# NumericalEarth/Breeze.jl

Hardware: AMD Instinct MI355X
Metric: grid-cells advanced/sec (tendency+Poisson step), 512^3 anelastic (higher is better)
Workload: dtype f64

## Files before the change

breeze.jl_amd/csrc/bz_tendency5.hip:

```cpp
#include <cstdlib>

#include "bz_tendency5_kernels.h"

__global__ void k_pi_dry(DevGrid g, double *__restrict__ pi, int n)
{
    const int t = blockIdx.x * blockDim.x + threadIdx.x;
    if (t >= n) return;
    const int k = t - g.Hz;
    const double q = 0.0, qd = 1.0 - q;
    const double Rm = qd * g.Rd + q * g.Rv;
    const double cpm = qd * g.cpd + q * g.cpv;
    pi[t] = pow(g.p_r[k] / g.pst, Rm / cpm);
}

__global__ void k_lev_rows(DevGrid g, const double *__restrict__ pi, LevRow5 *__restrict__ rows, int n)
{
    const int t = blockIdx.x * blockDim.x + threadIdx.x;
    if (t >= n) return;
    const int k = t - g.Hz;
    LevRow5 r;
    r.rho = g.rho[k]; r.rrho = g.rrho[k]; r.rho_f = g.rho_f[k]; r.rrho_f = g.rrho_f[k];
    r.Ax = g.Ax[k]; r.Ay = g.Ay[k]; r.Vinv_c = g.Vinv_c[k]; r.pi = pi[t];
    r.Vinv_f = g.Vinv_f[k]; r.T_r = g.T_r[k];
    for (int q = 0; q < 6; ++q) r.pad[q] = 0.0;
    rows[t] = r;
}

int bzi_lean_setup(bz_ctx *ctx)
{
    const DevGrid &g = ctx->dg;
    const int n = g.Nz + 2 * g.Hz;
    BZ_HIP(hipMalloc(&ctx->d_pi_dry, n * sizeof(double)));
    hipLaunchKernelGGL(k_pi_dry, dim3((n + 63) / 64), dim3(64), 0, 0, g, ctx->d_pi_dry, n);
    ctx->dg.pi_dry = ColPtr(ctx->d_pi_dry + g.Hz);
    BZ_HIP(hipMalloc(&ctx->d_lev_rows, n * sizeof(LevRow5)));
    hipLaunchKernelGGL(k_lev_rows, dim3((n + 63) / 64), dim3(64), 0, 0, g, ctx->d_pi_dry, (LevRow5 *)ctx->d_lev_rows, n);
    BZ_HIP(hipGetLastError());
    BZ_HIP(hipDeviceSynchronize());
    if (ctx->tune.side_cus > 0 && ctx->tune.side_cus < ctx->num_cus) {
        uint32_t mask[32] = {0};
        const int total = ctx->num_cus, want = ctx->tune.side_cus;
        for (int b = 0; b < want; ++b) {
            const int bit = ctx->tune.side_cu_layout == 1 ? (int)((long long)b * total / want) : b;
            mask[bit >> 5] |= 1u << (bit & 31);
        }
        BZ_HIP(hipExtStreamCreateWithCUMask(&ctx->side_stream, (uint32_t)((total + 31) / 32), mask));
    } else
    BZ_HIP(hipStreamCreateWithFlags(&ctx->side_stream, hipStreamNonBlocking));
    BZ_HIP(hipEventCreateWithFlags(&ctx->ev_fork, hipEventDisableTiming));
    BZ_HIP(hipEventCreateWithFlags(&ctx->ev_join, hipEventDisableTiming));
    ctx->side_scalar = ctx->tune.side_scalar;
    ctx->lean = !ctx->tune.no_lean;
    ctx->lean_xcd = !ctx->tune.no_xcd;
    return BZ_OK;
}

void bzi_lean_teardown(bz_ctx *ctx)
{
    if (ctx->d_pi_dry) hipFree(ctx->d_pi_dry);
    ctx->d_pi_dry = nullptr;
    if (ctx->d_lev_rows) hipFree(ctx->d_lev_rows);
    ctx->d_lev_rows = nullptr;
    if (ctx->d_qstate) hipFree(ctx->d_qstate);
    ctx->d_qstate = nullptr;
    if (ctx->h_qstate) hipHostFree(ctx->h_qstate);
    ctx->h_qstate = nullptr;
    if (ctx->ev_q) hipEventDestroy(ctx->ev_q);
    ctx->ev_q = nullptr;
    if (ctx->side_stream) { hipStreamSynchronize(ctx->side_stream); hipStreamDestroy(ctx->side_stream); ctx->side_stream = nullptr; }
    if (ctx->ev_fork) hipEventDestroy(ctx->ev_fork);
    if (ctx->ev_join) hipEventDestroy(ctx->ev_join);
    ctx->ev_fork = ctx->ev_join = nullptr;
}

static int pick_chunk5(const DevGrid &g, int nlev, int rows_per_block, bool fine = false)
{
    long long tiles = (long long)((g.Nx + 63) / 64) * ((g.Ny + rows_per_block - 1) / rows_per_block);
    const int floor_levels = fine ? 64 : 128;
    long long want = ((fine ? 4096 : 1024) + tiles - 1) / tiles;
    long long maxchunks = nlev / floor_levels > 0 ? nlev / floor_levels : 1;
    if (want > maxchunks) want = maxchunks;
    if (want < 1) want = 1;
    if (tiles * want < 512) {
        long long fill = (512 + tiles - 1) / tiles;
        long long cap = nlev / 8 > 0 ? nlev / 8 : 1;
        if (tiles * cap < 256) cap = nlev / 2 > 0 ? nlev / 2 : 1;
        if (fill > cap) fill = cap;
        if (fill > want) want = fill;
    }
    return (int)((nlev + want - 1) / want);
}

template <int TY>
static int lean_launch(bz_ctx *ctx, const bz_state *s, const bz_prognostic *U0, const bz_prognostic *G, const double *pa,
                       const double *pb, double *oa, double *ob, double dt, double alpha, bool first, int rows, int which)
{
    const DevGrid &g = ctx->dg;
    RKEpilogue E;
    E.mode = first ? 3 : 2; E.dt = dt; E.alpha = alpha; E.oma = 1.0 - alpha;
    Lean5 L;
    L.ru = s->rho_u; L.rv = s->rho_v; L.rw = s->rho_w; L.pa = pa; L.pb = pb; L.oa = oa; L.ob = ob; L.out = nullptr;
    L.T = s->T;
    L.pi_dry = ColPtr(ctx->d_pi_dry + g.Hz);
    L.lev = (const LevRow5 *)ctx->d_lev_rows + g.Hz;
    L.qstate = bzi_moisture_state(ctx);
    const int qh = L.qstate ? ctx->q_host : 2;
    L.mforce = 0; L.cor_f = 0.0; L.Fu = ColPtr(nullptr); L.Fv = ColPtr(nullptr); L.Su = ColPtr(nullptr); L.Sv = ColPtr(nullptr);
// ... 144 lines not shown
```

breeze.jl_amd/csrc/bz_tendency5_kernels.h:

```cpp
#pragma once
#include "bz_internal.h"
#include "bz_weno.h"
#include "bz_tendency4_kernels.h"

#ifndef BZ_KO
#define BZ_KO 0
#endif
#ifndef BZ6_ROTATE_DUTY
#define BZ6_ROTATE_DUTY 0
#endif
#ifndef BZ6_UNROLL2
#define BZ6_UNROLL2 0
#endif
#ifndef BZ6_LDS_BARRIER
#define BZ6_LDS_BARRIER 0
#endif
__device__ __forceinline__ void bz6_barrier()
{
#if BZ6_LDS_BARRIER
    __builtin_amdgcn_fence(__ATOMIC_RELEASE, "workgroup", "local");
    __builtin_amdgcn_s_barrier();
    __builtin_amdgcn_fence(__ATOMIC_ACQUIRE, "workgroup", "local");
#else
    __syncthreads();
#endif
}
typedef long long ix_t;
typedef unsigned ix32_t;

struct LevRow5 {
    double rho, rrho;
    double rho_f, rrho_f;
    double Ax, Ay, Vinv_c;
    double pi;
    double Vinv_f, T_r;
    double pad[6];
};
struct Lev5 {
    const LevRow5 *p;
#ifdef __HIPCC__
    __device__ __forceinline__ double at(int k, int f) const { return ((ColPtr::cptr)(const double *)p)[(long long)k * 16 + f]; }
    __device__ __forceinline__ double rho(int k) const { return at(k, 0); }
    __device__ __forceinline__ double rrho(int k) const { return at(k, 1); }
    __device__ __forceinline__ double rho_f(int k) const { return at(k, 2); }
    __device__ __forceinline__ double rrho_f(int k) const { return at(k, 3); }
    __device__ __forceinline__ double Ax(int k) const { return at(k, 4); }
    __device__ __forceinline__ double Ay(int k) const { return at(k, 5); }
    __device__ __forceinline__ double Vinv_c(int k) const { return at(k, 6); }
    __device__ __forceinline__ double pi(int k) const { return at(k, 7); }
    __device__ __forceinline__ double Vinv_f(int k) const { return at(k, 8); }
    __device__ __forceinline__ double T_r(int k) const { return at(k, 9); }
#endif
};
static_assert(sizeof(LevRow5) == 16 * sizeof(double), "LevRow5 is sixteen reals");

#ifndef BZ_LEAN_WAVES
#define BZ_LEAN_WAVES (sizeof(double) == 8 ? 4 : 6)
#endif
#ifndef BZ5_ZERO_SHORTCUT
#define BZ5_ZERO_SHORTCUT 1
#endif
#ifndef BZ5_TOPS_AHEAD
#define BZ5_TOPS_AHEAD 1
#endif
#ifndef BZ6_W_WAVES
#define BZ6_W_WAVES 4
#endif
#ifndef BZ5_EB
#define BZ5_EB 64
#endif
#ifndef BZ5_RAW_LDS
#define BZ5_RAW_LDS 0
#endif
#ifndef BZ5_SCALAR_WAVES
#define BZ5_SCALAR_WAVES (sizeof(double) == 8 ? 4 : 6)
#endif

struct Lean5 {
    const double *ru, *rv, *rw;
    const double *pa, *pb;
    double *out;
    double *oa, *ob;
    double *T;
    ColPtr pi_dry;
    const LevRow5 *lev;
    int mforce;
    double cor_f;
    ColPtr Fu, Fv;
    ColPtr Su, Sv;
    const double *vel, *bT, *bq;
    const int *qstate;
    int xcd;
    int by0, bys;
};

__device__ __forceinline__ void bz_block5(const Lean5 &L, int &bx, int &by, int &bz)
{
    bx = blockIdx.x; by = blockIdx.y; bz = blockIdx.z;
    if (L.xcd) {
        const unsigned gx = gridDim.x, gy = gridDim.y;
        const unsigned W = gx * gy * gridDim.z;
        unsigned w = bx + gx * (by + gy * bz);
        w = (w & 7u) * (W >> 3) + (w >> 3);
        bx = (int)(w % gx);
        by = (int)((w / gx) % gy);
        bz = (int)(w / (gx * gy));
    }
    by = L.by0 + by * L.bys;
    bx = __builtin_amdgcn_readfirstlane(bx);
    by = __builtin_amdgcn_readfirstlane(by);
    bz = __builtin_amdgcn_readfirstlane(bz);
}

__device__ __forceinline__ void st_img5(double *__restrict__ f, long long n, double v, long long ox, long long oy)
{
    f[n] = v;
    if (ox) f[n + ox] = v;
    if (oy) {
        f[n + oy] = v;
        if (ox) f[n + ox + oy] = v;
    }
}


__device__ __forceinline__ double bz_temperature5(const DevGrid &g, double rth, double rq, int k, const ColPtr pi_dry)
{
    const double rho = g.rho[k], rrho = g.rrho[k];
    const double th = bz_cdiv(rth, rho, rrho), q = bz_cdiv(rq, rho, rrho);
    if (pi_dry.p && __all(q == 0.0)) return pi_dry[k] * th;
    const double qd = 1.0 - q;
    const double cpm = qd * g.cpd + q * g.cpv;
    return bz_exner_factor(g, k, q, cpm) * th;
}

// ... 232 lines not shown
        }
        if (zz) fzb_hi = 0.0;
        else fzb_hi = (BZ_KO & 128) ? rf * (cfz * b[3]) : rf * (cfz * bz_upB(b[1], b[2], b[3], b[4], b[5], tb, lz, Bz));
        }
        double pa_n, pb_n;
        if constexpr (DRYQ) { pa_n = araw[0]; pb_n = b[3]; araw[0] = araw[1]; araw[1] = araw[2]; araw[2] = ta_raw; }
        else if (BZ_KO & 4) { pa_n = a[3]; pb_n = b[3]; }
        else if constexpr (BZ5_RAW_LDS) {
            double *ra = RAW + (lv3 * 2 + 0) * NT + t, *rb = ra + NT;
            pa_n = *ra; pb_n = *rb;
            *ra = ta_raw; *rb = tb_raw;
        } else { pa_n = pa[n]; pb_n = pb[n]; }
        T[buf ^ 1][0][ty + 3][tx + 3] = a[4];
        if constexpr (Q) T[buf ^ 1][1][ty + 3][tx + 3] = b[4];
        {
            const double rh = rho1, rr = rrho1;
            bool z1 = (b[4] == 0.0);
#pragma unroll
            for (int q = 0; q < HPT; ++q)
                if (hok[q]) {
                    T[buf ^ 1][0][hr[q]][hc[q]] = bz_cdiv(ha[q], rh, rr);
                    if constexpr (Q) {
                        const double hbv = bz_cdiv(hb[q], rh, rr);
                        T[buf ^ 1][1][hr[q]][hc[q]] = hbv;
                        z1 = z1 && (hbv == 0.0);
                    }
                }
            if (ZS && !__all(z1) && tx == 0) ZF[(lv3 + 1) % 3] = 0;
        }
        if (!(BZ_KO & 64)) __syncthreads();
        {
            double na = __shfl_down(fxa, 1);
            const double xa = __shfl(ea, src);
            if (tx == le) na = xa;
            const double dya = FY[buf][0][ty + 1][tx] - fya;
            const double Vi = Vi_k;
            const double ga = -(Vi * ((na - fxa) + dya + (fza_hi - fza)));
            double gb = 0.0;
            if constexpr (Q) {
                double nb = __shfl_down(fxb, 1);
                const double xb = __shfl(eb, src);
                if (tx == le) nb = xb;
                const double dyb = FY[buf][1][ty + 1][tx] - fyb;
                gb = -(Vi * ((nb - fxb) + dyb + (fzb_hi - fzb)));
            }
            if (store) {
                const double rth = bz_rk_apply_pre(E.mode, E.dt, E.alpha, E.oma, u0a, E.u0_out, ga, pa_n, n);
                F.oa[n] = rth;
                if constexpr (Q) {
                    const double rq = bz_rk_apply_pre(E.mode, E.dt, E.alpha, E.oma, u0b, E.u0b_out, gb, pb_n, n);
                    F.ob[n] = rq;
                }
            }
        }
        fza = fza_hi; fzb = fzb_hi;
#pragma unroll
        for (int s = 0; s < 5; ++s) { a[s] = a[s + 1]; b[s] = b[s + 1]; }
        a[5] = ta; b[5] = tb;
        buf ^= 1;
    }
}


template <bool DRYQ, bool GUARD>
__device__ __forceinline__ bool bz_lean_skip(const Lean5 &F)
{
    if constexpr (!GUARD) return false;
    const bool dry = F.qstate != nullptr && __builtin_amdgcn_readfirstlane(*F.qstate) == 1;
    return dry != DRYQ;
}
template <int TY, bool WY = false, bool DRYQ = false, bool GUARD = true>
__global__ __launch_bounds__(64 * TY) __attribute__((amdgpu_waves_per_eu(BZ5_SCALAR_WAVES, BZ5_SCALAR_WAVES))) void k5_scalar_pair(DevGrid g, Lean5 F, int kchunk, RKEpilogue E)
{
    constexpr int TR = TY + 6, TC = 72;
    __shared__ double T[2 * 2 * TR * TC];
    __shared__ double FY[2 * 2 * (TY + 1) * 64];
    __shared__ int ZF[3];
    __shared__ double RAW[(!DRYQ && BZ5_RAW_LDS) ? 3 * 2 * 64 * TY : 1];
    if (bz_lean_skip<DRYQ, GUARD>(F)) return;
    k5_scalar_pair_body<TY, WY, DRYQ>(g, F, kchunk, E, T, FY, ZF, RAW);
}

template <int KIND>
__device__ __forceinline__ double flux_x_lean(const DevGrid &g, const Tend3Fields &F, const double *__restrict__ m, int i, int j, int k, int By = 3)
{
    const long long n = g.idx(i, j, k);
    const double a = (KIND == T3_V && By != 3) ? bz_symm2(g.Ax[k] * F.ru[n - g.Sx], g.Ax[k] * F.ru[n]) : adv_x<KIND>(g, F, n, k);
    const double rh = (KIND == T3_W) ? g.rho_f[k] : g.rho[k], rr = (KIND == T3_W) ? g.rrho_f[k] : g.rrho[k];
    if constexpr (KIND == T3_U)
        return a * bz_up5(bz_cdiv(m[n - 2], rh, rr), bz_cdiv(m[n - 1], rh, rr), bz_cdiv(m[n], rh, rr), bz_cdiv(m[n + 1], rh, rr),
                          bz_cdiv(m[n + 2], rh, rr), bz_cdiv(m[n + 3], rh, rr), a > 0.0);
    else
        return a * bz_up5(bz_cdiv(m[n - 3], rh, rr), bz_cdiv(m[n - 2], rh, rr), bz_cdiv(m[n - 1], rh, rr), bz_cdiv(m[n], rh, rr),
                          bz_cdiv(m[n + 1], rh, rr), bz_cdiv(m[n + 2], rh, rr), a > 0.0);
}


template <int TY, bool MF = false, bool WY = false, bool ST = false>
__global__ __launch_bounds__(64 * TY, BZ_LEAN_WAVES) void k6_u(DevGrid g, Lean5 L, int kchunk, RKEpilogue E)
{
    static_assert(!(ST && WY), "stored-velocity instantiations: periodic / slab rows");
    constexpr int TR = TY + 6, TC = 72, NT = 64 * TY;
    constexpr int NH1 = TR * 70 - TY * 64;
    constexpr int NH2 = 3 * (TY + 1) + 64 + 3 * TY;
    static_assert(NH1 <= NT && NH2 <= NT, "one frame cell of each kind per thread");
    __shared__ double U[2][TR][TC];
    __shared__ double RU[2][TY][TC];
    __shared__ double RV[2][TY + 1][TC];
    __shared__ double RW[2][TY][TC];
    __shared__ double FY[2][TY + 1][64];
    int bx, by, bz;
    bz_block5(L, bx, by, bz);
    const int tx = threadIdx.x, ty = threadIdx.y, t = ty * 64 + tx, tc = tx + 3;
    const int i0 = bx * 64, j0 = by * TY;
    const int i = i0 + tx, j = j0 + ty;
    const int ic = min(i, g.Nx + 2), jc = min(j, g.Ny + 2);
    const int ie = i0 - 1, le = 0;
    const int kbeg = bz * kchunk, kend = min(kbeg + kchunk, g.Nz);
    if (kbeg >= kend) return;
    const ix_t sz = (ix_t)g.Sxy;
    const bool store = (i < g.Nx) && (j < g.Ny);
    const double *__restrict__ ru = L.ru, *__restrict__ rv = L.rv, *__restrict__ rw = L.rw;
    const double *__restrict__ vel = ST ? L.vel : L.ru;
    Tend3Fields F;
    F.ru = L.ru; F.rv = L.rv; F.rw = L.rw; F.u = F.v = F.w = F.T = F.q = nullptr; F.c = ST ? L.vel : nullptr; F.G = L.out;
    ix_t n = (ix_t)g.idx(ic, jc, kbeg);
    const bool h1ok = !(BZ_KO & 32768) && t < NH1;
    int h1r = 0, h1c = 0;
    {
        const int h = h1ok ? t : 0;
        if (h < 6 * 70) { const int rr = h / 70; h1c = h - rr * 70; h1r = (rr < 3) ? rr : TY + rr; }
        else { const int hh = h - 6 * 70, rr = hh / 6, cc = hh - rr * 6; h1r = 3 + rr; h1c = (cc < 3) ? cc : 64 + cc; }
    }
    const ix_t h1n = (ix_t)g.idx(min(i0 - 3 + h1c, g.Nx + 2), min(j0 - 3 + h1r, g.Ny + 2), kbeg);
    const bool h1raw = h1ok && h1r >= 3 && h1r < TY + 3 && (h1c == 2 || h1c == 67 || h1c == 68);
    const bool h2ok = !(BZ_KO & 32768) && t < NH2;
    int h2sel = 0, h2r = 0, h2c = 0;
    {
        const int id = h2ok ? t : 0;
        if (id < 3 * (TY + 1)) { h2r = id / 3; const int cc = id - 3 * h2r; h2c = (cc < 2) ? 1 + cc : 67; }
        else if (id < 3 * (TY + 1) + 64) { h2r = TY; h2c = 3 + (id - 3 * (TY + 1)); }
        else { h2sel = 1; const int m = id - 3 * (TY + 1) - 64; h2r = m / 3; const int cc = m - 3 * h2r; h2c = (cc < 2) ? 1 + cc : 67; }
    }
    const double *__restrict__ h2src = h2sel ? rw : rv;
    const ix_t h2n = (ix_t)g.idx(min(i0 - 3 + h2c, g.Nx + 2), min(j0 + h2r, g.Ny + 2), kbeg) + (h2sel ? sz : (ix_t)0);

    double r[6];
#pragma unroll
    for (int s = 0; s < 6; ++s) r[s] = ST ? vel[n + s * sz - 3 * sz] : bz_cdiv(ru[n + s * sz - 3 * sz], g.rho[kbeg + s - 3], g.rrho[kbeg + s - 3]);
    double fz_lo = vflux<T3_U>(g, F, n, kbeg, r[0], r[1], r[2], r[3], r[4], r[5]);
    double q0 = ru[n], q1 = ru[n + sz], q2 = ru[n + 2 * sz];
    U[0][ty + 3][tc] = r[3];
    RU[0][ty][tc] = q0;
    RV[0][ty][tc] = rv[n];
    RW[0][ty][tc] = rw[n + sz];
    if (h1ok) {
        const double raw = (ST && !h1raw) ? 0.0 : ru[h1n];
        U[0][h1r][h1c] = ST ? vel[h1n] : bz_cdiv(raw, g.rho[kbeg], g.rrho[kbeg]);
        if (h1raw) RU[0][h1r - 3][h1c] = raw;
    }
    if (h2ok) { if (h2sel) RW[0][h2r][h2c] = h2src[h2n]; else RV[0][h2r][h2c] = h2src[h2n]; }
    double tcur_raw = ru[n + 3 * sz];
    double tcur_v = ST ? vel[n + 3 * sz] : 0.0;
    double u0cur = (E.mode == 2) ? E.u0[n] : 0.0;
    __syncthreads();

    double edge = 0.0;
    int buf = 0;
#if BZ6_UNROLL2
#pragma unroll 2
#endif
    for (int k = kbeg; k < kend; ++k, n += sz) {
        const ix_t lev1 = (ix_t)(k + 1 - kbeg) * sz;
        const double p_top = ST ? ru[n + sz] : ru[n + ((k + 4 <= g.Nz + g.Hz - 1) ? 4 * sz : 3 * sz)];
        const double p_topv = ST ? vel[n + ((k + 4 <= g.Nz + g.Hz - 1) ? 4 * sz : 3 * sz)] : 0.0;
        const double p_h1 = (BZ_KO & 256) ? p_top : h1ok ? (ST ? vel : ru)[h1n + lev1] : 0.0;
        const double p_h1raw = (ST && h1raw) ? ru[h1n + lev1] : 0.0;
        const double p_h2 = (BZ_KO & 512) ? p_top : h2ok ? h2src[h2n + lev1] : 0.0;
        const double p_rv = (BZ_KO & 1024) ? p_top * 0.5 : rv[n + sz], p_rw = (BZ_KO & 1024) ? p_top * 0.25 : rw[n + 2 * sz];
        const double p_u0 = (BZ_KO & 2048) ? p_top : (E.mode == 2) ? E.u0[n + sz] : 0.0;
        if (((k - kbeg) & (BZ5_EB - 1)) == 0) {
            const int kk = min(k + (tx & (BZ5_EB - 1)), kend - 1);
            edge = ST ? flux_x_at<T3_U>(g, F, ie, jc, kk) : flux_x_lean<T3_U>(g, F, ru, ie, jc, kk);
        }
        const int src = (k - kbeg) & (BZ5_EB - 1);
        const double Ax = g.Ax[k], Ay = g.Ay[k], Az = g.Az;
        const double c0 = r[3];
        const double(*Uk)[TC] = U[buf];
        const double *rur = RU[buf][ty] + tc, *ur = Uk[ty + 3] + tc;
        const double ax = bz_symm4(Ax * rur[-1], Ax * q0, Ax * rur[1], Ax * rur[2]);
        const double fx = ax * bz_up5(ur[-2], ur[-1], c0, ur[1], ur[2], ur[3], ax > 0.0);
        const double *rvr = RV[buf][ty] + tc;
        const double ay = bz_symm4(Ay * rvr[-2], Ay * rvr[-1], Ay * rvr[0], Ay * rvr[1]);
        const double fy = ay * bz_up5y<WY>(Uk[ty][tc], Uk[ty + 1][tc], Uk[ty + 2][tc], c0, Uk[ty + 4][tc], Uk[ty + 5][tc], ay > 0.0, by5_face<WY>(g, __builtin_amdgcn_readfirstlane(j)));
        FY[buf][ty][tx] = fy;
        if (ty == (BZ6_ROTATE_DUTY ? ((k - kbeg) & (TY - 1)) : 0) && !(BZ_KO & 4096)) {
            const double *rvt = RV[buf][TY] + tc;
            const double at = bz_symm4(Ay * rvt[-2], Ay * rvt[-1], Ay * rvt[0], Ay * rvt[1]);
            FY[buf][TY][tx] = at * bz_up5y<WY>(Uk[TY][tc], Uk[TY + 1][tc], Uk[TY + 2][tc], Uk[TY + 3][tc], Uk[TY + 4][tc], Uk[TY + 5][tc], at > 0.0,
                                               by5_face<WY>(g, j0 + TY));
        }
        const double tnew = ST ? tcur_v : bz_cdiv(tcur_raw, g.rho[k + 3], g.rrho[k + 3]);
        const double *rwr = RW[buf][ty] + tc;
        const double wt = bz_symm4(Az * rwr[-2], Az * rwr[-1], Az * rwr[0], Az * rwr[1]);
        const double fz_hi = wt * bz_upB(r[1], r[2], r[3], r[4], r[5], tnew, wt > 0.0, bz_buffer_face(k + 1, g.Nz));
        U[buf ^ 1][ty + 3][tc] = r[4];
        RU[buf ^ 1][ty][tc] = ST ? p_top : q1;
        RV[buf ^ 1][ty][tc] = p_rv;
        RW[buf ^ 1][ty][tc] = p_rw;
        if (h1ok) {
            U[buf ^ 1][h1r][h1c] = ST ? p_h1 : bz_cdiv(p_h1, g.rho[k + 1], g.rrho[k + 1]);
            if (h1raw) RU[buf ^ 1][h1r - 3][h1c] = ST ? p_h1raw : p_h1;
        }
        if (h2ok) { if (h2sel) RW[buf ^ 1][h2r][h2c] = p_h2; else RV[buf ^ 1][h2r][h2c] = p_h2; }
        if (!(BZ_KO & 16384) && (!(BZ_KO & 8192) || ((k - kbeg) & 1))) bz6_barrier();
        {
            double nb = __shfl_up(fx, 1);
            const double e = __shfl(edge, src);
            if (tx == le) nb = e;
            const double dx = fx - nb;
            const double dy = (BZ_KO & 16384) ? 0.5 * fy : FY[buf][ty + 1][tx] - fy;
            double Gu = -(g.Vinv_c[k] * (dx + dy + (fz_hi - fz_lo)));
            if constexpr (MF) {
                if (L.mforce & 1) {
                    const double *rv0 = RV[buf][ty] + tc, *rv1 = RV[buf][ty + 1] + tc;
                    const double a = (rv0[-1] + rv1[-1]) / 2, b = (rv0[0] + rv1[0]) / 2;
                    Gu -= -L.cor_f * ((a + b) / 2);
                }
                if (L.mforce & (2 | 8)) {
                    const double rho = g.rho[k];
                    double tot = (L.mforce & 8) ? rho * L.Su[k] : 0.0;
                    if (L.mforce & 2) tot = (L.mforce & 8) ? tot + rho * L.Fu[k] : rho * L.Fu[k];
                    Gu += tot;
                }
            }
            if (store) L.out[n] = (ST && E.mode == 0) ? Gu : bz_rk_apply_pre(E.mode, E.dt, E.alpha, E.oma, u0cur, E.u0_out, Gu, q0, n);
        }
        fz_lo = fz_hi;
#pragma unroll
        for (int s = 0; s < 5; ++s) r[s] = r[s + 1];
        r[5] = tnew;
        if (ST) q0 = p_top;
        else { q0 = q1; q1 = q2; q2 = tcur_raw; tcur_raw = p_top; }
        u0cur = p_u0;
        if (ST) tcur_v = p_topv;
        buf ^= 1;
    }
}


template <int TY, bool MF = false, bool WY = false, bool ST = false>
__global__ __launch_bounds__(64 * TY, ((MF && WY) ? 4 : BZ_LEAN_WAVES)) void k6_v(DevGrid g, Lean5 L, int kchunk, RKEpilogue E)
{
    static_assert(!(ST && WY), "stored-velocity instantiations: periodic / slab rows");
    constexpr int RV = TY + 6, RM = TY + 4;
    constexpr int TC = 72;
    __shared__ double Tv[2][RV][TC];
    __shared__ double Tm[2][3][RM][64];
    __shared__ double FY[2][TY + 1][64];
    constexpr int NT = 64 * TY, NFR = 16 * 64, HPT = (NFR + NT - 1) / NT;
    int bx, by, bz;
    bz_block5(L, bx, by, bz);
    const int tx = threadIdx.x, ty = threadIdx.y, t = ty * 64 + tx, tc = tx + 3;
    const int i0 = bx * 64, j0 = by * TY;
    const int i = i0 + tx, j = j0 + ty;
    const int ic = min(i, g.Nx + 2), jc = min(j, g.Ny + 2);
    const int nact = min(64, g.Nx - i0);
    const int ie = i0 + nact, le = nact - 1;
    const int kbeg = bz * kchunk, kend = min(kbeg + kchunk, g.Nz);
    if (kbeg >= kend) return;
    const ix_t sz = (ix_t)g.Sxy;
    const bool store = (i < g.Nx) && (j < g.Ny) && !(WY && j == 0);
    const int ju = __builtin_amdgcn_readfirstlane(j);
    const int Bf = by5_face<WY>(g, ju), Bc = by5_center<WY>(g, ju), Bc0 = by5_center<WY>(g, j0 - 1);
    const double *__restrict__ ru = L.ru, *__restrict__ rv = L.rv, *__restrict__ rw = L.rw;
    const double *__restrict__ vel = ST ? L.vel : L.rv;
    Tend3Fields F;
    F.ru = L.ru; F.rv = L.rv; F.rw = L.rw; F.u = F.v = F.w = F.T = F.q = nullptr; F.c = ST ? L.vel : nullptr; F.G = L.out;
    const double Az = g.Az;
    ix_t n = (ix_t)g.idx(ic, jc, kbeg);

    bool hok[HPT];
    int hsel[HPT], hrow[HPT];
    ix_t hn[HPT];
    const double *hsrc[HPT];
#pragma unroll
    for (int q = 0; q < HPT; ++q) {
        const int h = t + q * NT;
        hok[q] = h < NFR;
        const int id = __builtin_amdgcn_readfirstlane(hok[q] ? (h >> 6) : 0);
        int sel, row, grow;
        if (id < 6) { sel = 0; row = (id < 3) ? id : TY + id; grow = j0 - 3 + row; }
        else if (id < 9) { sel = 1; const int m = id - 6; row = (m < 2) ? m : TY + 2; grow = j0 - 2 + row; }
        else if (id < 13) { sel = 2; const int m = id - 9; row = (m < 2) ? m : TY + m; grow = j0 - 2 + row; }
        else { sel = 3; const int m = id - 13; row = (m < 2) ? m : TY + 2; grow = j0 - 2 + row; }
        hsel[q] = sel; hrow[q] = row;
        hsrc[q] = (sel == 1) ? ru : (sel == 3) ? rw : (ST && sel == 0) ? vel : rv;
        hn[q] = (ix_t)g.idx(min(i0 + tx, g.Nx + 2), min(grow, g.Ny + 2), kbeg) + (sel == 3 ? sz : (ix_t)0);
    }
    auto frame_load = [&](int q, ix_t lev) -> double { return hsrc[q][hn[q] + lev]; };
    auto frame_store = [&](int b, int q, double raw, int klev) {
        if (hsel[q] == 0) Tv[b][hrow[q]][tc] = ST ? raw : bz_cdiv(raw, g.rho[klev], g.rrho[klev]);
        else Tm[b][hsel[q] - 1][hrow[q]][tx] = ((hsel[q] == 1) ? g.Ax[klev] : (hsel[q] == 2) ? g.Ay[klev] : Az) * raw;
    };

    const bool sok = t < 5 * TY;
    const int srow = sok ? t / 5 : 0, scc = sok ? t % 5 : 0, scol = (scc < 3) ? scc : 64 + scc;
    const ix_t sn = (ix_t)g.idx(min(i0 - 3 + scol, g.Nx + 2), min(j0 + srow, g.Ny + 2), kbeg);

    double r[6];
#pragma unroll
    for (int s = 0; s < 6; ++s) r[s] = ST ? vel[n + s * sz - 3 * sz] : bz_cdiv(rv[n + s * sz - 3 * sz], g.rho[kbeg + s - 3], g.rrho[kbeg + s - 3]);
    double fz_lo;
    if (WY && Bf != 3) {
        const double wt0 = bz_symm2(Az * rw[n - (ix_t)g.Sx], Az * rw[n]);
        fz_lo = wt0 * bz_upB(r[0], r[1], r[2], r[3], r[4], r[5], wt0 > 0.0, bz_buffer_face(kbeg, g.Nz));
    } else fz_lo = vflux<T3_V>(g, F, n, kbeg, r[0], r[1], r[2], r[3], r[4], r[5]);
    double q0 = rv[n], q1 = rv[n + sz], q2 = rv[n + 2 * sz];
    Tv[0][ty + 3][tc] = r[3];
    if (sok) Tv[0][srow + 3][scol] = ST ? vel[sn] : bz_cdiv(rv[sn], g.rho[kbeg], g.rrho[kbeg]);
    Tm[0][0][ty + 2][tx] = g.Ax[kbeg] * ru[n];
    Tm[0][1][ty + 2][tx] = g.Ay[kbeg] * q0;
    Tm[0][2][ty + 2][tx] = Az * rw[n + sz];
#pragma unroll
    for (int q = 0; q < HPT; ++q)
        if (hok[q]) frame_store(0, q, frame_load(q, 0), kbeg);
    __syncthreads();

    double tcur_raw = rv[n + 3 * sz];
// ... 8 lines not shown
        for (int q = 0; q < HPT; ++q) hnext[q] = hok[q] ? frame_load(q, lev) : 0.0;
        const double p_side = sok ? (ST ? vel : rv)[sn + lev] : 0.0;
        const double p_top = ST ? rv[n + sz] : rv[n + ((k + 4 <= g.Nz + g.Hz - 1) ? 4 * sz : 3 * sz)];
        const double p_topv = ST ? vel[n + ((k + 4 <= g.Nz + g.Hz - 1) ? 4 * sz : 3 * sz)] : 0.0;
        const double p_u0 = (E.mode == 2) ? E.u0[n + sz] : 0.0;
        const double tnew_raw = tcur_raw, u0v = u0cur;
        const double ru_n = g.Ax[k + 1] * ru[n + sz], rw_n = Az * rw[n + 2 * sz];
        double cor_u = 0.0, cg1 = 0.0, cg3 = 0.0;
        if constexpr (MF) { if ((L.mforce & 1) && tx == 63) { const ix_t sy = (ix_t)g.Sx; cg1 = ru[n - sy + 1]; cg3 = ru[n + 1]; } }
        if (((k - kbeg) & (BZ5_EB - 1)) == 0) {
            const int kk = min(k + (tx & (BZ5_EB - 1)), kend - 1);
            edge = ST ? flux_x_at<T3_V>(g, F, ie, jc, kk) : flux_x_lean<T3_V>(g, F, rv, ie, jc, kk, Bf);
        }
        const int src = (k - kbeg) & (BZ5_EB - 1);
        const double rho = g.rho[k];
        const double c0 = r[3];
        const double(*V)[TC] = Tv[buf];
        const double *vrow = V[ty + 3] + tc;
        const double(*MU)[64] = Tm[buf][0];
        const double(*MV)[64] = Tm[buf][1];
        const double(*MW)[64] = Tm[buf][2];
        const double ut = bz_symm4y<WY>(MU[ty][tx], MU[ty + 1][tx], MU[ty + 2][tx], MU[ty + 3][tx], Bf);
        const double fx = ut * bz_up5(vrow[-3], vrow[-2], vrow[-1], c0, vrow[1], vrow[2], ut > 0.0);
        const double vt = (!WY || Bc == 3) ? bz_symm4(MV[ty + 1][tx], MV[ty + 2][tx], MV[ty + 3][tx], MV[ty + 4][tx]) : bz_symm2(MV[ty + 2][tx], MV[ty + 3][tx]);
        const double fy = vt * bz_up5y<WY>(V[ty + 1][tc], V[ty + 2][tc], c0, V[ty + 4][tc], V[ty + 5][tc], V[ty + 6][tc], vt > 0.0, Bc);
        FY[buf][ty + 1][tx] = fy;
        if (ty == 0 && !(BZ_KO & 4096)) {
            const double vb = (!WY || Bc0 == 3) ? bz_symm4(MV[0][tx], MV[1][tx], MV[2][tx], MV[3][tx]) : bz_symm2(MV[1][tx], MV[2][tx]);
            FY[buf][0][tx] = vb * bz_up5y<WY>(V[0][tc], V[1][tc], V[2][tc], V[3][tc], V[4][tc], V[5][tc], vb > 0.0, Bc0);
        }
        const double tnew = ST ? tcur_v : bz_cdiv(tnew_raw, g.rho[k + 3], g.rrho[k + 3]);
        const double wt = bz_symm4y<WY>(MW[ty][tx], MW[ty + 1][tx], MW[ty + 2][tx], MW[ty + 3][tx], Bf);
        const double fz_hi = wt * bz_upB(r[1], r[2], r[3], r[4], r[5], tnew, wt > 0.0, bz_buffer_face(k + 1, g.Nz));
        if constexpr (MF) {
            if (L.mforce & 1) {
                const double Axk = g.Ax[k];
                const double l1 = MU[ty + 1][tx + 1], l3 = MU[ty + 2][tx + 1];
                const double c1 = (tx == 63) ? Axk * cg1 : l1, c3 = (tx == 63) ? Axk * cg3 : l3;
                cor_u = (((MU[ty + 1][tx] + c1) / 2 + (MU[ty + 2][tx] + c3) / 2) / 2) / Axk;
            }
        }
        Tv[buf ^ 1][ty + 3][tc] = r[4];
        if (sok) Tv[buf ^ 1][srow + 3][scol] = ST ? p_side : bz_cdiv(p_side, g.rho[k + 1], g.rrho[k + 1]);
        Tm[buf ^ 1][0][ty + 2][tx] = ru_n;
        Tm[buf ^ 1][1][ty + 2][tx] = g.Ay[k + 1] * (ST ? p_top : q1);
        Tm[buf ^ 1][2][ty + 2][tx] = rw_n;
#pragma unroll
        for (int q = 0; q < HPT; ++q)
            if (hok[q]) frame_store(buf ^ 1, q, hnext[q], k + 1);
        bz6_barrier();
        {
            double nb = __shfl_down(fx, 1);
            const double e = __shfl(edge, src);
            if (tx == le) nb = e;
            const double dx = nb - fx;
            const double dy = fy - FY[buf][ty][tx];
            double Gv = -(g.Vinv_c[k] * (dx + dy + (fz_hi - fz_lo)));
            if constexpr (MF) {
                if (L.mforce & 1) Gv -= L.cor_f * cor_u;
                if (L.mforce & (4 | 16)) {
                    double tot = (L.mforce & 16) ? rho * L.Sv[k] : 0.0;
                    if (L.mforce & 4) tot = (L.mforce & 16) ? tot + rho * L.Fv[k] : rho * L.Fv[k];
                    Gv += tot;
                }
            }
            if (store) L.out[n] = (ST && E.mode == 0) ? Gv : bz_rk_apply_pre(E.mode, E.dt, E.alpha, E.oma, u0v, E.u0_out, Gv, q0, n);
            if constexpr (WY) {
                if (i < g.Nx && j == 0) L.out[n] = 0.0;
                if (i < g.Nx && j == g.Ny - 1) L.out[n + (ix_t)g.Sx] = 0.0;
            }
        }
        fz_lo = fz_hi;
        if (ST) q0 = p_top;
        else { q0 = q1; q1 = q2; q2 = tnew_raw; tcur_raw = p_top; }
        u0cur = p_u0;
        if (ST) tcur_v = p_topv;
#pragma unroll
        for (int s = 0; s < 5; ++s) r[s] = r[s + 1];
        r[5] = tnew;
        buf ^= 1;
    }
}

__device__ __forceinline__ double buoyancy5(const DevGrid &g, double rth, double rq, int k, double rho, double rrho, double pi, double T_ref)
{
    const double th = bz_cdiv(rth, rho, rrho), q = bz_cdiv(rq, rho, rrho);
    double T;
    if (__all(q == 0.0)) T = pi * th;
    else {
        const double qd = 1.0 - q;
        const double cpm = qd * g.cpd + q * g.cpv;
        T = bz_exner_factor(g, k, q, cpm) * th;
    }
    const double Rm = (1.0 - q) * g.Rd + q * g.Rv;
    const double rhop = rho * (g.Rd * T_ref / (Rm * T) - 1.0);
    return -g.g * rhop;
}


template <int TY, bool WY = false, bool DRYQ = false, bool GUARD = true, int BM = 4>
__global__ __launch_bounds__(64 * TY, BZ6_W_WAVES) void k6_w(DevGrid g, Lean5 L, int kchunk, RKEpilogue E)
{
    constexpr bool ST = BM != 4;
    static_assert(!(ST && (WY || DRYQ || GUARD)), "stored-velocity instantiations: periodic / slab rows, no moisture-scan dispatch");
    if (bz_lean_skip<DRYQ, GUARD>(L)) return;
    constexpr int TR = TY + 6, TC = 72, NT = 64 * TY, NH = TR * 70 - TY * 64;
    static_assert(NH <= NT, "one frame cell per thread");
    __shared__ double T[2][TR][TC];
    __shared__ double FY[2][TY + 1][64];
    int bx, by, bz;
    bz_block5(L, bx, by, bz);
    const int tx = threadIdx.x, ty = threadIdx.y, t = ty * 64 + tx, tc = tx + 3;
    const int i0 = bx * 64, j0 = by * TY;
    const int i = i0 + tx, j = j0 + ty;
    const int ic = min(i, g.Nx + 2), jc = min(j, g.Ny + 2);
    const int nact = min(64, g.Nx - i0);
    const int ie = i0 + nact, le = nact - 1;
    const int kbeg = 1 + bz * kchunk, kend = min(kbeg + kchunk, g.Nz);
    if (kbeg >= kend) return;
    const ix32_t sz = (ix32_t)g.Sxy;
    const bool store = (i < g.Nx) && (j < g.Ny);
    const double *__restrict__ ru = L.ru, *__restrict__ rv = L.rv, *__restrict__ rw = L.rw;
    const double *__restrict__ pa = L.pa, *__restrict__ pb = L.pb;
    const double *__restrict__ vel = ST ? L.vel : L.rw;
    const double *__restrict__ bT = L.bT, *__restrict__ bq = L.bq;
    const Lev5 LV{L.lev};
    constexpr bool dryq = DRYQ;
    Tend3Fields F;
    F.ru = L.ru; F.rv = L.rv; F.rw = L.rw; F.u = F.v = F.w = F.T = F.q = nullptr; F.c = ST ? L.vel : nullptr; F.G = L.out;
    const double Az = g.Az;
    ix32_t n = (ix32_t)g.idx(ic, jc, kbeg);
    const bool hok = t < NH;
    int hr = 0, hc = 0;
    {
        const int h = hok ? t : 0;
        if (h < 6 * 70) { const int rr = h / 70; hc = h - rr * 70; hr = (rr < 3) ? rr : TY + rr; }
        else { const int hh = h - 6 * 70, rr = hh / 6, cc = hh - rr * 6; hr = 3 + rr; hc = (cc < 3) ? cc : 64 + cc; }
    }
    const ix32_t hn = (ix32_t)g.idx(min(i0 - 3 + hc, g.Nx + 2), min(j0 - 3 + hr, g.Ny + 2), kbeg);
    const ix32_t ntop0 = (ix32_t)g.idx(ic, min(j0 + TY, g.Ny), kbeg);
    const bool top = (ty == 0);

    double wr[6], qu[4], qv[4], qt[4], qw[4];
    double raw0 = 0.0, raw1 = 0.0, raw2 = 0.0;
#pragma unroll
    for (int s = 0; s < 6; ++s) {
        const double x = rw[n + s * sz - 3 * sz];
        wr[s] = ST ? vel[n + s * sz - 3 * sz] : bz_cdiv(x, LV.rho_f(kbeg + s - 3), LV.rrho_f(kbeg + s - 3));
        if (s >= 1 && s <= 4) qw[s - 1] = Az * x;
        if (s == 3) raw0 = x;
        if (s == 4) raw1 = x;
        if (s == 5) raw2 = x;
    }
#pragma unroll
    for (int s = 0; s < 4; ++s) {
        const int kk = kbeg - 2 + s;
        const double Axk = ST ? g.Ax[kk] : LV.Ax(kk), Ayk = ST ? g.Ay[kk] : LV.Ay(kk);
        qu[s] = Axk * ru[n + s * sz - 2 * sz];
        qv[s] = Ayk * rv[n + s * sz - 2 * sz];
        qt[s] = top ? Ayk * rv[ntop0 + s * sz - 2 * sz] : 0.0;
    }
    double fz_lo, b_lo, r_lo = 0.0;
    {
        const int B = bz_buffer_center(kbeg - 1, g.Nz);
        const double wt = (B == 3) ? bz_symm4(qw[0], qw[1], qw[2], qw[3]) : bz_symm2(qw[1], qw[2]);
        fz_lo = wt * bz_upB(wr[0], wr[1], wr[2], wr[3], wr[4], wr[5], wt > 0.0, B);
        if constexpr (BM == 4) b_lo = buoyancy5(g, pa[n - sz], dryq ? 0.0 : pb[n - sz], kbeg - 1, LV.rho(kbeg - 1), LV.rrho(kbeg - 1), LV.pi(kbeg - 1), LV.T_r(kbeg - 1));
        else if constexpr (BM == 0) b_lo = buoyancy3(g, bT[n - sz], bq[n - sz], kbeg - 1);
        else if constexpr (BM == 3) b_lo = bz_buoyancy(g, bT, bq, (long long)(n - sz), kbeg - 1);
        else if constexpr (BM == 2) { b_lo = bT[n - sz] - g.p_r[kbeg - 1]; r_lo = bq[n - sz] - g.rho[kbeg - 1]; }
        else b_lo = 0.0;
    }
    T[0][ty + 3][tc] = wr[3];
    if (hok) T[0][hr][hc] = ST ? vel[hn] : bz_cdiv(rw[hn], LV.rho_f(kbeg), LV.rrho_f(kbeg));
    double tcur_raw = rw[n + 3 * sz];
    double tcur_v = ST ? vel[n + 3 * sz] : 0.0;
    double u0cur = (E.mode == 2) ? E.u0[n] : 0.0;
    __syncthreads();

    double edge = 0.0;
    int buf = 0;
    for (int k = kbeg; k < kend; ++k, n += sz) {
        const ix32_t lev = (ix32_t)(k - kbeg) * sz;
        const double p_h = hok ? (ST ? vel : rw)[hn + lev + sz] : 0.0;
        const double p_top = rw[n + ((k + 4 <= g.Nz + g.Hz) ? 4 * sz : 3 * sz)];
        const double p_topv = ST ? vel[n + ((k + 4 <= g.Nz + g.Hz) ? 4 * sz : 3 * sz)] : 0.0;
        const double Tcur = (BM == 1) ? 0.0 : (ST ? bT : pa)[n], rqcur = (BM == 1) ? 0.0 : ST ? bq[n] : dryq ? 0.0 : pb[n];
        const double p_u0 = (E.mode == 2) ? E.u0[n + sz] : 0.0;
        const double Axn = ST ? g.Ax[k + 2] : LV.Ax(k + 2), Ayn = ST ? g.Ay[k + 2] : LV.Ay(k + 2);
        const double qun = Axn * ru[n + 2 * sz], qvn = Ayn * rv[n + 2 * sz];
        const double qtn = top ? Ayn * rv[ntop0 + lev + 2 * sz] : 0.0;
        if (((k - kbeg) & (BZ5_EB - 1)) == 0) {
            const int kk = min(k + (tx & (BZ5_EB - 1)), kend - 1);
            edge = ST ? flux_x_at<T3_W>(g, F, ie, jc, kk) : flux_x_lean<T3_W>(g, F, rw, ie, jc, kk);
        }
        const int src = (k - kbeg) & (BZ5_EB - 1);
        const int Bf = bz_buffer_face(k, g.Nz);
        const double w0 = wr[3];
        const double qwnew = Az * (ST ? rw[n + 2 * sz] : raw2);
        const double uold = ST ? rw[n] : raw0;
        const double(*Tk)[TC] = T[buf];
        const double *wrow = Tk[ty + 3] + tc;
        const double ut = (Bf == 3) ? bz_symm4(qu[0], qu[1], qu[2], qu[3]) : bz_symm2(qu[1], qu[2]);
        const double fx = ut * bz_up5(wrow[-3], wrow[-2], wrow[-1], w0, wrow[1], wrow[2], ut > 0.0);
        const double vt = (Bf == 3) ? bz_symm4(qv[0], qv[1], qv[2], qv[3]) : bz_symm2(qv[1], qv[2]);
        const double fy = vt * bz_up5y<WY>(Tk[ty][tc], Tk[ty + 1][tc], Tk[ty + 2][tc], w0, Tk[ty + 4][tc], Tk[ty + 5][tc], vt > 0.0, by5_face<WY>(g, __builtin_amdgcn_readfirstlane(j)));
        FY[buf][ty][tx] = fy;
        if (top && !(BZ_KO & 4096)) {
            const double v2 = (Bf == 3) ? bz_symm4(qt[0], qt[1], qt[2], qt[3]) : bz_symm2(qt[1], qt[2]);
            FY[buf][TY][tx] = v2 * bz_up5y<WY>(Tk[TY][tc], Tk[TY + 1][tc], Tk[TY + 2][tc], Tk[TY + 3][tc], Tk[TY + 4][tc], Tk[TY + 5][tc], v2 > 0.0,
                                               by5_face<WY>(g, j0 + TY));
        }
        const double wnew = ST ? tcur_v : bz_cdiv(tcur_raw, LV.rho_f(k + 3), LV.rrho_f(k + 3));
        double fz_hi;
        {
            const int B = bz_buffer_center(k, g.Nz);
            const double wt = (B == 3) ? bz_symm4(qw[1], qw[2], qw[3], qwnew) : bz_symm2(qw[2], qw[3]);
            fz_hi = wt * bz_upB(wr[1], wr[2], wr[3], wr[4], wr[5], wnew, wt > 0.0, B);
        }
        double b_hi = 0.0, r_hi = 0.0;
        if constexpr (BM == 4) b_hi = buoyancy5(g, Tcur, rqcur, k, LV.rho(k), LV.rrho(k), LV.pi(k), LV.T_r(k));
        else if constexpr (BM == 0) b_hi = buoyancy3(g, Tcur, rqcur, k);
        else if constexpr (BM == 3) b_hi = bz_buoyancy(g, bT, bq, (long long)n, k);
        else if constexpr (BM == 2) { b_hi = Tcur - g.p_r[k]; r_hi = rqcur - g.rho[k]; }
        T[buf ^ 1][ty + 3][tc] = wr[4];
        if (hok) T[buf ^ 1][hr][hc] = ST ? p_h : bz_cdiv(p_h, LV.rho_f(k + 1), LV.rrho_f(k + 1));
        bz6_barrier();
        {
            double nb = __shfl_down(fx, 1);
            const double e = __shfl(edge, src);
            if (tx == le) nb = e;
            const double dx = nb - fx;
            const double dy = FY[buf][ty + 1][tx] - fy;
            const double adv = -((ST ? g.Vinv_f[k] : LV.Vinv_f(k)) * (dx + dy + (fz_hi - fz_lo)));
            double Gval;
            if constexpr (BM == 2) Gval = adv - (b_hi - b_lo) * g.rdzf[k] - g.g * ((r_hi + r_lo) / 2.0);
            else if constexpr (BM == 1) Gval = adv;
            else Gval = adv + 0.5 * (b_lo + b_hi);
            if (store)
                L.out[n] = (ST && E.mode == 0) ? Gval : bz_rk_apply_pre(E.mode, E.dt, E.alpha, E.oma, u0cur, E.u0_out, Gval, uold, n);
        }
        fz_lo = fz_hi;
        b_lo = b_hi;
        r_lo = r_hi;
#pragma unroll
        for (int s = 0; s < 3; ++s) { qu[s] = qu[s + 1]; qv[s] = qv[s + 1]; qt[s] = qt[s + 1]; qw[s] = qw[s + 1]; }
        qu[3] = qun; qv[3] = qvn; qt[3] = qtn; qw[3] = qwnew;
        raw0 = raw1; raw1 = raw2; raw2 = tcur_raw;
        tcur_raw = p_top; u0cur = p_u0;
        if (ST) tcur_v = p_topv;
#pragma unroll
        for (int s = 0; s < 5; ++s) wr[s] = wr[s + 1];
        wr[5] = wnew;
        buf ^= 1;
    }
}
```

Before: 4.191 billion.

## Unroll u-kernel vertical loop by two and specialize dry buoyancy with cached ln(pi)

The u-momentum kernel's vertical sweep is manually unrolled by two for the plain periodic variant. Stencil registers are indexed by phase modulo six and three, so the per-level shift of the r and q windows becomes a rotation once per pair of levels. The buoyancy routine gets a compile-time dry specialization that skips moisture work. The moist path now uses a precomputed ln(pi) column, stored in the padded level row, in place of the Exner factor call, and the edge flux index is derived from the current linear index rather than recomputed. These changes aim to cut register moves and arithmetic, but the unroll may raise register pressure and the mod-indexed arrays rely on full unrolling to stay in registers.

```diff
diff --git a/breeze.jl_amd/csrc/bz_tendency5.hip b/breeze.jl_amd/csrc/bz_tendency5.hip
--- a/breeze.jl_amd/csrc/bz_tendency5.hip
+++ b/breeze.jl_amd/csrc/bz_tendency5.hip
@@ -21,8 +21,8 @@
     LevRow5 r;
     r.rho = g.rho[k]; r.rrho = g.rrho[k]; r.rho_f = g.rho_f[k]; r.rrho_f = g.rrho_f[k];
     r.Ax = g.Ax[k]; r.Ay = g.Ay[k]; r.Vinv_c = g.Vinv_c[k]; r.pi = pi[t];
-    r.Vinv_f = g.Vinv_f[k]; r.T_r = g.T_r[k];
-    for (int q = 0; q < 6; ++q) r.pad[q] = 0.0;
+    r.Vinv_f = g.Vinv_f[k]; r.T_r = g.T_r[k]; r.lnpi = g.lnpi[k];
+    for (int q = 0; q < 5; ++q) r.pad[q] = 0.0;
     rows[t] = r;
 }
 
diff --git a/breeze.jl_amd/csrc/bz_tendency5_kernels.h b/breeze.jl_amd/csrc/bz_tendency5_kernels.h
--- a/breeze.jl_amd/csrc/bz_tendency5_kernels.h
+++ b/breeze.jl_amd/csrc/bz_tendency5_kernels.h
@@ -8,9 +8,6 @@
 #endif
 #ifndef BZ6_ROTATE_DUTY
 #define BZ6_ROTATE_DUTY 0
-#endif
-#ifndef BZ6_UNROLL2
-#define BZ6_UNROLL2 0
 #endif
 #ifndef BZ6_LDS_BARRIER
 #define BZ6_LDS_BARRIER 0
@@ -34,7 +31,8 @@
     double Ax, Ay, Vinv_c;
     double pi;
     double Vinv_f, T_r;
-    double pad[6];
+    double lnpi;
+    double pad[5];
 };
 struct Lev5 {
     const LevRow5 *p;
@@ -50,6 +48,7 @@
     __device__ __forceinline__ double pi(int k) const { return at(k, 7); }
     __device__ __forceinline__ double Vinv_f(int k) const { return at(k, 8); }
     __device__ __forceinline__ double T_r(int k) const { return at(k, 9); }
+    __device__ __forceinline__ double lnpi(int k) const { return at(k, 10); }
 #endif
 };
 static_assert(sizeof(LevRow5) == 16 * sizeof(double), "LevRow5 is sixteen reals");
@@ -448,9 +447,15 @@
 }
 
 template <int KIND>
+__device__ __forceinline__ double flux_x_lean_at(const DevGrid &g, const Tend3Fields &F, const double *__restrict__ m, long long n, int k, int By = 3);
+template <int KIND>
 __device__ __forceinline__ double flux_x_lean(const DevGrid &g, const Tend3Fields &F, const double *__restrict__ m, int i, int j, int k, int By = 3)
 {
-    const long long n = g.idx(i, j, k);
+    return flux_x_lean_at<KIND>(g, F, m, g.idx(i, j, k), k, By);
+}
+template <int KIND>
+__device__ __forceinline__ double flux_x_lean_at(const DevGrid &g, const Tend3Fields &F, const double *__restrict__ m, long long n, int k, int By)
+{
     const double a = (KIND == T3_V && By != 3) ? bz_symm2(g.Ax[k] * F.ru[n - g.Sx], g.Ax[k] * F.ru[n]) : adv_x<KIND>(g, F, n, k);
     const double rh = (KIND == T3_W) ? g.rho_f[k] : g.rho[k], rr = (KIND == T3_W) ? g.rrho_f[k] : g.rrho[k];
     if constexpr (KIND == T3_U)
@@ -515,9 +520,9 @@
 #pragma unroll
     for (int s = 0; s < 6; ++s) r[s] = ST ? vel[n + s * sz - 3 * sz] : bz_cdiv(ru[n + s * sz - 3 * sz], g.rho[kbeg + s - 3], g.rrho[kbeg + s - 3]);
     double fz_lo = vflux<T3_U>(g, F, n, kbeg, r[0], r[1], r[2], r[3], r[4], r[5]);
-    double q0 = ru[n], q1 = ru[n + sz], q2 = ru[n + 2 * sz];
+    double q[3] = {ru[n], ru[n + sz], ru[n + 2 * sz]};
     U[0][ty + 3][tc] = r[3];
-    RU[0][ty][tc] = q0;
+    RU[0][ty][tc] = q[0];
     RV[0][ty][tc] = rv[n];
     RW[0][ty][tc] = rw[n + sz];
     if (h1ok) {
@@ -533,10 +538,12 @@
 
     double edge = 0.0;
     int buf = 0;
-#if BZ6_UNROLL2
-#pragma unroll 2
-#endif
-    for (int k = kbeg; k < kend; ++k, n += sz) {
+    constexpr int GL = (!MF && !WY && !ST) ? 2 : 1;
+    for (int k0 = kbeg; k0 < kend; k0 += GL) {
+#pragma unroll
+    for (int ph = 0; ph < GL; ++ph) {
+        const int k = k0 + ph;
+        if (k >= kend) break;
         const ix_t lev1 = (ix_t)(k + 1 - kbeg) * sz;
         const double p_top = ST ? ru[n + sz] : ru[n + ((k + 4 <= g.Nz + g.Hz - 1) ? 4 * sz : 3 * sz)];
         const double p_topv = ST ? vel[n + ((k + 4 <= g.Nz + g.Hz - 1) ? 4 * sz : 3 * sz)] : 0.0;
@@ -551,10 +558,10 @@
         }
         const int src = (k - kbeg) & (BZ5_EB - 1);
         const double Ax = g.Ax[k], Ay = g.Ay[k], Az = g.Az;
-        const double c0 = r[3];
+        const double c0 = r[(3 + ph) % 6];
         const double(*Uk)[TC] = U[buf];
         const double *rur = RU[buf][ty] + tc, *ur = Uk[ty + 3] + tc;
-        const double ax = bz_symm4(Ax * rur[-1], Ax * q0, Ax * rur[1], Ax * rur[2]);
+        const double ax = bz_symm4(Ax * rur[-1], Ax * q[ph % 3], Ax * rur[1], Ax * rur[2]);
         const double fx = ax * bz_up5(ur[-2], ur[-1], c0, ur[1], ur[2], ur[3], ax > 0.0);
         const double *rvr = RV[buf][ty] + tc;
         const double ay = bz_symm4(Ay * rvr[-2], Ay * rvr[-1], Ay * rvr[0], Ay * rvr[1]);
@@ -569,9 +576,9 @@
         const double tnew = ST ? tcur_v : bz_cdiv(tcur_raw, g.rho[k + 3], g.rrho[k + 3]);
         const double *rwr = RW[buf][ty] + tc;
         const double wt = bz_symm4(Az * rwr[-2], Az * rwr[-1], Az * rwr[0], Az * rwr[1]);
-        const double fz_hi = wt * bz_upB(r[1], r[2], r[3], r[4], r[5], tnew, wt > 0.0, bz_buffer_face(k + 1, g.Nz));
-        U[buf ^ 1][ty + 3][tc] = r[4];
-        RU[buf ^ 1][ty][tc] = ST ? p_top : q1;
+        const double fz_hi = wt * bz_upB(r[(1 + ph) % 6], r[(2 + ph) % 6], r[(3 + ph) % 6], r[(4 + ph) % 6], r[(5 + ph) % 6], tnew, wt > 0.0, bz_buffer_face(k + 1, g.Nz));
+        U[buf ^ 1][ty + 3][tc] = r[(4 + ph) % 6];
+        RU[buf ^ 1][ty][tc] = ST ? p_top : q[(1 + ph) % 3];
         RV[buf ^ 1][ty][tc] = p_rv;
         RW[buf ^ 1][ty][tc] = p_rw;
         if (h1ok) {
@@ -600,17 +607,28 @@
                     Gu += tot;
                 }
             }
-            if (store) L.out[n] = (ST && E.mode == 0) ? Gu : bz_rk_apply_pre(E.mode, E.dt, E.alpha, E.oma, u0cur, E.u0_out, Gu, q0, n);
+            if (store) L.out[n] = (ST && E.mode == 0) ? Gu : bz_rk_apply_pre(E.mode, E.dt, E.alpha, E.oma, u0cur, E.u0_out, Gu, q[ph % 3], n);
         }
         fz_lo = fz_hi;
-#pragma unroll
-        for (int s = 0; s < 5; ++s) r[s] = r[s + 1];
-        r[5] = tnew;
-        if (ST) q0 = p_top;
-        else { q0 = q1; q1 = q2; q2 = tcur_raw; tcur_raw = p_top; }
+        r[ph % 6] = tnew;
+        if (ST) q[(1 + ph) % 3] = p_top;
+        else { q[ph % 3] = tcur_raw; tcur_raw = p_top; }
         u0cur = p_u0;
         if (ST) tcur_v = p_topv;
         buf ^= 1;
+        n += sz;
+    }
+    {
+        double t6[6], t3[3];
+#pragma unroll
+        for (int s = 0; s < 6; ++s) t6[s] = r[(s + GL) % 6];
+#pragma unroll
+        for (int s = 0; s < 6; ++s) r[s] = t6[s];
+#pragma unroll
+        for (int s = 0; s < 3; ++s) t3[s] = q[(s + GL) % 3];
+#pragma unroll
+        for (int s = 0; s < 3; ++s) q[s] = t3[s];
+    }
     }
 }
 
@@ -785,15 +803,21 @@
     }
 }
 
-__device__ __forceinline__ double buoyancy5(const DevGrid &g, double rth, double rq, int k, double rho, double rrho, double pi, double T_ref)
-{
+template <bool DRY>
+__device__ __forceinline__ double buoyancy5(const DevGrid &g, double rth, double rq, double rho, double rrho, double pi, double lnpi, double T_ref)
+{
+    if constexpr (DRY) {
+        const double T = pi * bz_cdiv(rth, rho, rrho);
+        const double rhop = rho * (g.Rd * T_ref / (g.Rd * T) - 1.0);
+        return -g.g * rhop;
+    }
     const double th = bz_cdiv(rth, rho, rrho), q = bz_cdiv(rq, rho, rrho);
     double T;
     if (__all(q == 0.0)) T = pi * th;
     else {
         const double qd = 1.0 - q;
         const double cpm = qd * g.cpd + q * g.cpv;
-        T = bz_exner_factor(g, k, q, cpm) * th;
+        T = (pi * bz_exp_small(((q * g.kap_num) / (cpm * g.cpd)) * lnpi)) * th;
     }
     const double Rm = (1.0 - q) * g.Rd + q * g.Rv;
     const double rhop = rho * (g.Rd * T_ref / (Rm * T) - 1.0);
@@ -868,7 +892,7 @@
         const int B = bz_buffer_center(kbeg - 1, g.Nz);
         const double wt = (B == 3) ? bz_symm4(qw[0], qw[1], qw[2], qw[3]) : bz_symm2(qw[1], qw[2]);
         fz_lo = wt * bz_upB(wr[0], wr[1], wr[2], wr[3], wr[4], wr[5], wt > 0.0, B);
-        if constexpr (BM == 4) b_lo = buoyancy5(g, pa[n - sz], dryq ? 0.0 : pb[n - sz], kbeg - 1, LV.rho(kbeg - 1), LV.rrho(kbeg - 1), LV.pi(kbeg - 1), LV.T_r(kbeg - 1));
+        if constexpr (BM == 4) b_lo = buoyancy5<dryq>(g, pa[n - sz], dryq ? 0.0 : pb[n - sz], LV.rho(kbeg - 1), LV.rrho(kbeg - 1), LV.pi(kbeg - 1), dryq ? 0.0 : LV.lnpi(kbeg - 1), LV.T_r(kbeg - 1));
         else if constexpr (BM == 0) b_lo = buoyancy3(g, bT[n - sz], bq[n - sz], kbeg - 1);
         else if constexpr (BM == 3) b_lo = bz_buoyancy(g, bT, bq, (long long)(n - sz), kbeg - 1);
         else if constexpr (BM == 2) { b_lo = bT[n - sz] - g.p_r[kbeg - 1]; r_lo = bq[n - sz] - g.rho[kbeg - 1]; }
@@ -895,7 +919,9 @@
         const double qtn = top ? Ayn * rv[ntop0 + lev + 2 * sz] : 0.0;
         if (((k - kbeg) & (BZ5_EB - 1)) == 0) {
             const int kk = min(k + (tx & (BZ5_EB - 1)), kend - 1);
-            edge = ST ? flux_x_at<T3_W>(g, F, ie, jc, kk) : flux_x_lean<T3_W>(g, F, rw, ie, jc, kk);
+            if constexpr (ST) edge = flux_x_at<T3_W>(g, F, ie, jc, kk);
+            else if constexpr (DRYQ) edge = flux_x_lean<T3_W>(g, F, rw, ie, jc, kk);
+            else edge = flux_x_lean_at<T3_W>(g, F, rw, (long long)n + (ie - min(i, g.Nx + 2)) + (long long)(kk - k) * sz, kk);
         }
         const int src = (k - kbeg) & (BZ5_EB - 1);
         const int Bf = bz_buffer_face(k, g.Nz);
@@ -922,7 +948,7 @@
             fz_hi = wt * bz_upB(wr[1], wr[2], wr[3], wr[4], wr[5], wnew, wt > 0.0, B);
         }
         double b_hi = 0.0, r_hi = 0.0;
-        if constexpr (BM == 4) b_hi = buoyancy5(g, Tcur, rqcur, k, LV.rho(k), LV.rrho(k), LV.pi(k), LV.T_r(k));
+        if constexpr (BM == 4) b_hi = buoyancy5<dryq>(g, Tcur, rqcur, LV.rho(k), LV.rrho(k), LV.pi(k), dryq ? 0.0 : LV.lnpi(k), LV.T_r(k));
         else if constexpr (BM == 0) b_hi = buoyancy3(g, Tcur, rqcur, k);
         else if constexpr (BM == 3) b_hi = bz_buoyancy(g, bT, bq, (long long)n, k);
         else if constexpr (BM == 2) { b_hi = Tcur - g.p_r[k]; r_hi = rqcur - g.rho[k]; }
```

Result: no change. 4.216 billion, median of 6 (+0.6%).
